# jhhung/kISS

Measured on AMD Instinct MI355X. Metric: bases/sec suffix_sort (chm13v2.0-size synthetic, k=256), higher is better.
Workload: dtype u8; 1 GPU; suffix_sort genome-like synthetic n=3117292070 k=256 (stand-in for chm13v2.0.fa, BASELINE.json configs[1]); PARALLEL_SORTING; text resident in HBM, SA left in HBM; n=3117292070, k=256, seed=2, parallelism=single GPU, lms=905939973, lms_rounds=9, tied_after_round0_item_rounds=184319413, big_segment_item_rounds=72866550, workspace_bytes=80357006484, induce_passes=47

## Files before the change

kiss_amd/csrc/induce.hip:

```cpp
#include "kiss_internal.hpp"
#include <cstdio>
#include <cstdlib>

namespace {

constexpr int IN_THREADS = 256;
#ifndef KISS_IN_ITEMS
#define KISS_IN_ITEMS 8
#endif
constexpr int IN_ITEMS = KISS_IN_ITEMS;
constexpr int IN_WAVES = IN_THREADS / 64;
constexpr int IN_TILE = IN_THREADS * IN_ITEMS;
constexpr int SM_THREADS = 1024;
constexpr uint64_t SMALL_MAX = 8192;

__device__ __forceinline__ uint32_t child_ctx(uint32_t parent)
{
    return (KISS_CTX_WORD(parent) >> 2) | (parent & KISS_CTX_TAINT);
}

__device__ __forceinline__ uint32_t cls_byte(uint32_t c)
{
    return (c & 3u) | ((c & 0x7FFFFFFEu) == 0u ? 4u : 0u);
}
static_assert(KISS_EMPTY_CTX == 1u && KISS_CTX_TAINT == 0x80000000u, "no bases <=> all bits but 0 and 31 clear");

struct LmsRemap {
    const uint32_t *fin;
    const uint32_t *npos;
    uint32_t E;
};

__device__ __forceinline__ uint32_t remap_below(const LmsRemap &rm, uint64_t j)
{
    uint32_t lo = 0, hi = rm.E;
    while (lo < hi) {
        const uint32_t mid = (lo + hi) >> 1;
        if ((uint64_t)rm.fin[mid] < j) lo = mid + 1;
        else hi = mid;
    }
    return lo;
}

__device__ __forceinline__ uint32_t remap_below_wave(const LmsRemap &rm, uint64_t j)
{
    if (rm.E > 256u) return remap_below(rm, j);
    uint32_t cnt = 0;
    for (uint32_t base = 0; base < rm.E; base += 64u) {
        const uint32_t i = base + lane_id();
        const bool lt = i < rm.E && (uint64_t)rm.fin[i] < j;
        const uint32_t c = (uint32_t)__popcll(__ballot(lt));
        cnt += c;
        if (c < 64u) break;
    }
    return cnt;
}

template <bool REMAP>
__device__ __forceinline__ uint32_t item_class(const uint64_t *__restrict__ pk, const uint32_t *srcP, uint32_t *srcC,
                                               int64_t idx, uint32_t emitmask, uint32_t *v_out, uint32_t *ctx_out,
                                               const LmsRemap &rm, uint8_t *srcK = nullptr)
{
    int64_t phys = idx;
    if (REMAP) {
        const uint32_t t = remap_below(rm, (uint64_t)idx);
        if (t < rm.E && (int64_t)rm.fin[t] == idx) {
            const uint32_t v = rm.npos[t];
            const uint32_t c = kiss_load_ctx(pk, v) | KISS_CTX_TAINT;
            *v_out = v;
            *ctx_out = c;
            const uint32_t pc = c & 3u;
            return (v != 0 && ((emitmask >> pc) & 1u)) ? pc : 4u;
        }
        phys = idx - (int64_t)t;
    }
    uint32_t c = srcC[phys];
    uint32_t v = srcP[phys];
    *v_out = v;
    if (KISS_CTX_WORD(c) <= KISS_EMPTY_CTX) {
        if (v == 0) {
            *ctx_out = c;
            return 4u;
        }
        c = kiss_load_ctx(pk, v) | (c & KISS_CTX_TAINT);
        srcC[phys] = c;
        if (srcK) srcK[phys] = (uint8_t)cls_byte(c);
    }
    *ctx_out = c;
    uint32_t pc = c & 3u;
    return ((emitmask >> pc) & 1u) ? pc : 4u;
}

template <bool REMAP>
__device__ __forceinline__ uint32_t item_class_only(const uint64_t *__restrict__ pk, const uint32_t *srcP, uint32_t *srcC,
                                                    int64_t idx, uint32_t emitmask, const LmsRemap &rm, uint8_t *srcK = nullptr)
{
    if (REMAP) {
        uint32_t v, c;
        return item_class<true>(pk, srcP, srcC, idx, emitmask, &v, &c, rm);
    }
    uint32_t c = srcC[idx];
    if (KISS_CTX_WORD(c) <= KISS_EMPTY_CTX) {
        const uint32_t v = srcP[idx];
        if (v == 0) return 4u;
        c = kiss_load_ctx(pk, v) | (c & KISS_CTX_TAINT);
        srcC[idx] = c;
        if (srcK) srcK[idx] = (uint8_t)cls_byte(c);
    }
    const uint32_t pc = c & 3u;
    return ((emitmask >> pc) & 1u) ? pc : 4u;
}

__device__ __forceinline__ uint32_t wave_scan_add(uint32_t x)
{
    x += (uint32_t)__builtin_amdgcn_update_dpp(0, (int)x, 0x111, 0xf, 0xf, true);
    x += (uint32_t)__builtin_amdgcn_update_dpp(0, (int)x, 0x112, 0xf, 0xf, true);
    x += (uint32_t)__builtin_amdgcn_update_dpp(0, (int)x, 0x114, 0xf, 0xf, true);
    x += (uint32_t)__builtin_amdgcn_update_dpp(0, (int)x, 0x118, 0xf, 0xf, true);
    x += (uint32_t)__builtin_amdgcn_update_dpp(0, (int)x, 0x142, 0xa, 0xf, true);
    x += (uint32_t)__builtin_amdgcn_update_dpp(0, (int)x, 0x143, 0xc, 0xf, true);
    return x;
}

template <bool REMAP>
__global__ __launch_bounds__(IN_THREADS) void k_induce_count(const uint64_t *__restrict__ pk, const uint32_t *srcP,
                                                            uint32_t *srcC, int64_t beg, uint64_t N, int dir,
                                                            uint32_t emitmask, uint32_t *__restrict__ counts,
                                                            uint64_t tiles, LmsRemap rm, uint8_t *srcK)
{
    if (blockIdx.x == 0 && threadIdx.x == 4) counts[4 * tiles] = 0;
    const uint64_t tile = (uint64_t)blockIdx.x * IN_WAVES + (threadIdx.x >> 6);
    if (tile >= tiles) return;
    struct __attribute__((packed, aligned(4))) U4 {
        uint32_t v[4];
    };
    constexpr int STEPS = IN_TILE / 256;
    const uint32_t lane = lane_id();
    const uint64_t t0 = tile * IN_TILE;
    uint64_t acc = 0;
    int64_t shift = 0;
    bool block = t0 + IN_TILE <= N;
    if (REMAP && block) {
        const uint32_t b0 = remap_below_wave(rm, (uint64_t)beg + t0);
        block = b0 == remap_below_wave(rm, (uint64_t)beg + t0 + IN_TILE);
        shift = (int64_t)b0;
    }
    bool counted = false;
    if (!REMAP && srcK != nullptr && block) {
        const int64_t lo_index = dir > 0 ? beg + (int64_t)t0 : beg - (int64_t)(t0 + IN_TILE - 1);
        const uint8_t *const A = srcK + lo_index;
        const uint32_t mis = (uint32_t)(reinterpret_cast<uintptr_t>(A) & 15u);
        const uint4 *const ap = reinterpret_cast<const uint4 *>(A - mis);
        static_assert(IN_TILE == 2048, "64 lanes x 2 x 16 bytes");
        uint32_t w[12];
        {
            const uint4 q0 = ap[lane], q1 = ap[64 + lane];
            w[0] = q0.x, w[1] = q0.y, w[2] = q0.z, w[3] = q0.w;
            w[4] = q1.x, w[5] = q1.y, w[6] = q1.z, w[7] = q1.w;
            w[8] = w[9] = w[10] = w[11] = 0x08080808u;
        }
        if (mis != 0 && lane == 0) {
            const uint4 q2 = ap[128];
            const uint32_t tail[4] = {q2.x, q2.y, q2.z, q2.w};
#pragma unroll
            for (int i = 0; i < 4; i++) {
                const int nb = (int)mis - 4 * i;
                const uint32_t lowmask = nb >= 4 ? 0xFFFFFFFFu : (nb <= 0 ? 0u : ~(0xFFFFFFFFu << (8 * nb)));
                w[i] = (w[i] & ~lowmask) | (0x08080808u & lowmask);
                w[8 + i] = (tail[i] & lowmask) | (0x08080808u & ~lowmask);
            }
        }
        uint32_t any = 0;
#pragma unroll
        for (int i = 0; i < 12; i++) any |= w[i];
        if (__ballot((any & 0x04040404u) != 0u) == 0ull) {
            uint32_t cnt8 = 0;
#pragma unroll
            for (int i = 0; i < 12; i++) {
#pragma unroll
                for (int e = 0; e < 4; e++) {
                    const uint32_t b = (w[i] >> (8 * e)) & 0xFFu;
                    const uint32_t pc = b & 3u;
                    cnt8 += ((emitmask >> pc) & ~(b >> 3) & 1u) << (pc << 3);
                }
            }
            acc = (uint64_t)((cnt8 & 0xFFu) | ((cnt8 & 0xFF00u) << 8)) | ((uint64_t)(((cnt8 >> 16) & 0xFFu) | ((cnt8 >> 8) & 0xFF0000u)) << 32);
            counted = true;
        }
    }
    if (counted) {
    } else if (block) {
        U4 t[STEPS];
        int64_t p0[STEPS];
        uint32_t least = 0xFFFFFFFFu;
#pragma unroll
        for (int q = 0; q < STEPS; q++) {
            const uint64_t i0 = t0 + (uint64_t)q * 256 + 4 * lane;
            p0[q] = (dir > 0 ? beg + (int64_t)i0 : beg - (int64_t)(i0 + 3)) - shift;
            t[q] = *reinterpret_cast<const U4 *>(srcC + p0[q]);
        }
#pragma unroll
        for (int q = 0; q < STEPS; q++)
#pragma unroll
            for (int e = 0; e < 4; e++) least = min(least, t[q].v[e] & 0x7FFFFFFEu);
        uint32_t cnt8 = 0;
        if (__ballot(least == 0u) == 0ull) {
#pragma unroll
            for (int q = 0; q < STEPS; q++) {
#pragma unroll
                for (int e = 0; e < 4; e++) {
                    const uint32_t pc = t[q].v[e] & 3u;
                    cnt8 += ((emitmask >> pc) & 1u) << (pc << 3);
                }
            }
        } else {
#pragma unroll
            for (int q = 0; q < STEPS; q++) {
#pragma unroll
                for (int e = 0; e < 4; e++) {
                    const uint32_t c = t[q].v[e];
                    uint32_t cls;
                    if (KISS_CTX_WORD(c) <= KISS_EMPTY_CTX) cls = item_class_only<false>(pk, srcP, srcC, p0[q] + e, emitmask, rm, REMAP ? nullptr : srcK);
                    else {
                        const uint32_t pc = c & 3u;
                        cls = ((emitmask >> pc) & 1u) ? pc : 4u;
                    }
                    cnt8 += (cls < 4u ? 1u : 0u) << ((cls & 3u) << 3);
                }
            }
        }
        static_assert(IN_TILE / 64 <= 255, "8-bit counters per lane");
        acc = (uint64_t)((cnt8 & 0xFFu) | ((cnt8 & 0xFF00u) << 8)) | ((uint64_t)(((cnt8 >> 16) & 0xFFu) | ((cnt8 >> 8) & 0xFF0000u)) << 32);
    } else {
        for (uint64_t i = t0 + lane; i < N && i < t0 + IN_TILE; i += 64) {
            const uint32_t cls = item_class_only<REMAP>(pk, srcP, srcC, beg + (int64_t)dir * (int64_t)i, emitmask, rm, REMAP ? nullptr : srcK);
            acc += cls < 4u ? 1ull << (16 * cls) : 0ull;
        }
    }
    const uint32_t slo = (uint32_t)__builtin_amdgcn_readlane((int)wave_scan_add((uint32_t)acc), 63);
    const uint32_t shi = (uint32_t)__builtin_amdgcn_readlane((int)wave_scan_add((uint32_t)(acc >> 32)), 63);
    acc = ((uint64_t)shi << 32) | slo;
    if (lane < 4) counts[(uint64_t)lane * tiles + tile] = (uint32_t)(acc >> (16 * lane)) & 0xFFFFu;
}

struct DstPos {
    int64_t p[4];
};

template <bool REMAP, int DIR>
__global__ __launch_bounds__(IN_THREADS) void k_induce_scatter(const uint64_t *__restrict__ pk, const uint32_t *srcP,
                                                              uint32_t *srcC, int64_t beg, uint64_t N,
                                                              uint32_t emitmask, const uint32_t *__restrict__ ex,
                                                              uint64_t tiles, DstPos dst, uint32_t *SA, uint32_t *CTX,
                                                              uint32_t *__restrict__ totals, LmsRemap rm,
                                                              uint8_t *CLS,
                                                              uint8_t *srcK)
{
    static_assert(IN_ITEMS == 8 && IN_WAVES == 4, "8-bit counters per thread, 4-bit ranks of a thread's items in one word");
    static_assert(!REMAP || DIR > 0, "the LMS list is read left to right only");
    __shared__ uint32_t wtot[IN_WAVES][2];
    __shared__ __attribute__((aligned(16))) uint32_t stP[IN_TILE];
    __shared__ __attribute__((aligned(16))) uint32_t stC[IN_TILE];
    if (blockIdx.x == 0 && threadIdx.x < 4) totals[threadIdx.x] = ex[(uint64_t)(threadIdx.x + 1) * tiles] - ex[(uint64_t)threadIdx.x * tiles];
    const int wave = threadIdx.x >> 6;
    struct __attribute__((packed, aligned(4))) U4 {
        uint32_t v[4];
    };
    const uint64_t i0 = (uint64_t)blockIdx.x * IN_TILE + (uint64_t)threadIdx.x * IN_ITEMS;
    uint32_t vv[IN_ITEMS], cc[IN_ITEMS];
    uint32_t okm = 0;
    uint32_t loc = 0;
    uint32_t cnt8 = 0;
    auto take = [&](int e, uint32_t pc, uint32_t ok) {
        const uint32_t sh = pc << 3;
        loc |= ((cnt8 >> sh) & 15u) << (4 * e);
        cnt8 += ok << sh;
        okm |= ok << e;
    };
    int64_t shift = 0;
    bool block = i0 + IN_ITEMS <= N;
    if (REMAP) {
        const uint64_t tj = (uint64_t)beg + (uint64_t)blockIdx.x * IN_TILE;
        const uint32_t t0 = remap_below_wave(rm, tj), t1 = remap_below_wave(rm, tj + IN_TILE);
        if (t0 == t1) shift = (int64_t)t0;
        else if (block) {
            const uint32_t b0 = remap_below(rm, (uint64_t)beg + i0);
            block = b0 == remap_below(rm, (uint64_t)beg + i0 + IN_ITEMS);
            shift = (int64_t)b0;
        }
    }
    if (block) {
        const int64_t p0 = (DIR > 0 ? beg + (int64_t)i0 : beg - (int64_t)(i0 + IN_ITEMS - 1)) - shift;
        uint32_t bp[IN_ITEMS], bc[IN_ITEMS];
#pragma unroll
        for (int q = 0; q < IN_ITEMS / 4; q++) {
            const U4 tp = *reinterpret_cast<const U4 *>(srcP + p0 + 4 * q);
            const U4 tcw = *reinterpret_cast<const U4 *>(srcC + p0 + 4 * q);
#pragma unroll
            for (int e = 0; e < 4; e++) {
                bp[4 * q + e] = tp.v[e];
                bc[4 * q + e] = tcw.v[e];
            }
        }
        uint32_t least = 0xFFFFFFFFu;
#pragma unroll
        for (int e = 0; e < IN_ITEMS; e++) least = min(least, bc[e] & 0x7FFFFFFEu);
        static_assert(KISS_EMPTY_CTX == 1u && KISS_CTX_TAINT == 0x80000000u, "no bases <=> all bits but 0 and 31 clear");
        constexpr int last = IN_ITEMS - 1;
        if (__ballot(least == 0u) == 0ull) {
#pragma unroll
            for (int e = 0; e < IN_ITEMS; e++) {
                const int a = DIR > 0 ? e : last - e;
                const uint32_t pc = bc[a] & 3u;
                take(e, pc, (emitmask >> pc) & 1u);
                vv[e] = bp[a];
                cc[e] = bc[a];
            }
        } else {
#pragma unroll
            for (int e = 0; e < IN_ITEMS; e++) {
                const int a = DIR > 0 ? e : last - e;
                uint32_t v = bp[a], c = bc[a];
                if (KISS_CTX_WORD(c) <= KISS_EMPTY_CTX) {
                    const uint32_t cls = item_class<false>(pk, srcP, srcC, p0 + a, emitmask, &v, &c, rm, REMAP ? nullptr : srcK);
                    take(e, cls & 3u, cls < 4u ? 1u : 0u);
                } else {
                    const uint32_t pc = c & 3u;
                    take(e, pc, (emitmask >> pc) & 1u);
                }
                vv[e] = v;
                cc[e] = c;
            }
        }
    } else {
#pragma unroll
        for (int e = 0; e < IN_ITEMS; e++) {
            const uint64_t i = i0 + (uint64_t)e;
            uint32_t cls = 4u, v = 0, c = 0;
            if (i < N) cls = item_class<REMAP>(pk, srcP, srcC, beg + (int64_t)DIR * (int64_t)i, emitmask, &v, &c, rm, REMAP ? nullptr : srcK);
            take(e, cls & 3u, cls < 4u ? 1u : 0u);
            vv[e] = v;
            cc[e] = c;
        }
    }
    const uint32_t mylo = (cnt8 & 0xFFu) | ((cnt8 & 0xFF00u) << 8), myhi = ((cnt8 >> 16) & 0xFFu) | ((cnt8 >> 8) & 0xFF0000u);
    const uint32_t inlo = wave_scan_add(mylo), inhi = wave_scan_add(myhi);
    if (lane_id() == 63) {
        wtot[wave][0] = inlo;
        wtot[wave][1] = inhi;
    }
    __syncthreads();
    uint32_t tlo = 0, thi = 0, olo = 0, ohi = 0;
#pragma unroll
    for (int w = 0; w < IN_WAVES; w++) {
        const uint32_t a = wtot[w][0], b = wtot[w][1];
        tlo += a;
        thi += b;
        if (w < wave) {
            olo += a;
            ohi += b;
        }
    }
    const uint32_t c1 = tlo & 0xFFFFu, c2 = c1 + (tlo >> 16), c3 = c2 + (thi & 0xFFFFu), total = c3 + (thi >> 16);
    const uint32_t blo = (c1 << 16) + olo + (inlo - mylo), bhi = (c2 | (c3 << 16)) + ohi + (inhi - myhi);
#pragma unroll
    for (int e = 0; e < IN_ITEMS; e++) {
        if ((okm >> e) & 1u) {
            const uint32_t pc = cc[e] & 3u;
            const uint32_t base = __builtin_amdgcn_perm(bhi, blo, 0x0c0c0100u + pc * 0x0202u);
            const uint32_t li = base + ((loc >> (4 * e)) & 15u);
            stP[li] = vv[e] - 1u;
            stC[li] = child_ctx(cc[e]);
        }
    }
    __syncthreads();
    int64_t db[4];
    {
        const uint32_t cs[4] = {0u, c1, c2, c3};
#pragma unroll
        for (int k = 0; k < 4; k++) {
            const uint32_t toff = ex[(uint64_t)k * tiles + blockIdx.x] - ex[(uint64_t)k * tiles];
            db[k] = dst.p[k] + (int64_t)DIR * ((int64_t)toff - (int64_t)cs[k]);
        }
    }
    for (uint32_t l0 = threadIdx.x * 4u; l0 < total; l0 += IN_THREADS * 4u) {
        const uint32_t cls = (l0 >= c1 ? 1u : 0u) + (l0 >= c2 ? 1u : 0u) + (l0 >= c3 ? 1u : 0u);
        const uint32_t cend = cls == 0 ? c1 : (cls == 1 ? c2 : (cls == 2 ? c3 : total));
        if (l0 + 4u <= cend) {
            const int64_t dbk = cls == 0 ? db[0] : (cls == 1 ? db[1] : (cls == 2 ? db[2] : db[3]));
            const int64_t d0 = dbk + (int64_t)DIR * (int64_t)l0;
            const uint4 sp = *reinterpret_cast<const uint4 *>(stP + l0), sc = *reinterpret_cast<const uint4 *>(stC + l0);
            U4 wp, wc;
            if (DIR > 0) {
                wp.v[0] = sp.x, wp.v[1] = sp.y, wp.v[2] = sp.z, wp.v[3] = sp.w;
                wc.v[0] = sc.x, wc.v[1] = sc.y, wc.v[2] = sc.z, wc.v[3] = sc.w;
            } else {
                wp.v[0] = sp.w, wp.v[1] = sp.z, wp.v[2] = sp.y, wp.v[3] = sp.x;
                wc.v[0] = sc.w, wc.v[1] = sc.z, wc.v[2] = sc.y, wc.v[3] = sc.x;
            }
            const int64_t lo = DIR > 0 ? d0 : d0 - 3;
            *reinterpret_cast<U4 *>(SA + lo) = wp;
            *reinterpret_cast<U4 *>(CTX + lo) = wc;
            if (CLS) {
                struct __attribute__((packed, aligned(1))) B4 {
                    uint32_t v;
                };
                reinterpret_cast<B4 *>(CLS + lo)->v =
                    cls_byte(wc.v[0]) | (cls_byte(wc.v[1]) << 8) | (cls_byte(wc.v[2]) << 16) | (cls_byte(wc.v[3]) << 24);
            }
        } else {
            for (uint32_t li = l0; li < l0 + 4u && li < total; li++) {
                const uint32_t c2_ = (li >= c1 ? 1u : 0u) + (li >= c2 ? 1u : 0u) + (li >= c3 ? 1u : 0u);
                const int64_t dbk = c2_ == 0 ? db[0] : (c2_ == 1 ? db[1] : (c2_ == 2 ? db[2] : db[3]));
                const int64_t d = dbk + (int64_t)DIR * (int64_t)li;
                SA[d] = stP[li];
                CTX[d] = stC[li];
                if (CLS) CLS[d] = (uint8_t)cls_byte(stC[li]);
            }
        }
    }
}

constexpr uint32_t IN_SPIN_LIMIT = 1u << 22;
static_assert(IN_WAVES == 4, "wave c of a partition tile walks class c");

__device__ __forceinline__ uint32_t in_lookback(uint64_t *__restrict__ d, uint32_t tile, uint32_t mine, uint64_t tag,
                                                uint32_t *__restrict__ err)
{
    const uint32_t lane = lane_id();
    constexpr uint64_t TAGMASK = 0x3FFFFFFFull << 32;
    if (tile == 0) {
        if (lane == 0) __hip_atomic_store(&d[0], (2ull << 62) | tag | mine, __ATOMIC_RELAXED, __HIP_MEMORY_SCOPE_AGENT);
        return 0u;
    }
    if (lane == 0) __hip_atomic_store(&d[tile], (1ull << 62) | tag | mine, __ATOMIC_RELAXED, __HIP_MEMORY_SCOPE_AGENT);
    uint32_t excl = 0, spins = 0;
    int64_t base = (int64_t)tile;
    for (;;) {
        const int64_t t = base - 1 - (int64_t)lane;
        uint64_t v = t >= 0 ? __hip_atomic_load(&d[t], __ATOMIC_RELAXED, __HIP_MEMORY_SCOPE_AGENT) : ((2ull << 62) | tag);
        if ((v & TAGMASK) != tag) v = 0;
        const uint32_t st = (uint32_t)(v >> 62);
        const uint64_t incl = __ballot(st == 2u), ready = __ballot(st != 0u);
        const uint32_t first = incl ? (uint32_t)__builtin_ctzll(incl) : 64u;
        const uint64_t need = first >= 63u ? ~0ull : ((2ull << first) - 1ull);
        if ((ready & need) != need) {
            if (++spins > IN_SPIN_LIMIT) {
                if (lane == 0) *err = 1;
                break;
            }
            __builtin_amdgcn_s_sleep(1);
            continue;
        }
        uint32_t a = lane <= first ? (uint32_t)v : 0u;
#pragma unroll
        for (int dd = 32; dd >= 1; dd >>= 1) a += __shfl_xor(a, dd, 64);
        excl += a;
        if (first < 64u) break;
        base -= 64;
    }
    if (lane == 0) __hip_atomic_store(&d[tile], (2ull << 62) | tag | (uint64_t)(uint32_t)(excl + mine), __ATOMIC_RELAXED, __HIP_MEMORY_SCOPE_AGENT);
    return excl;
}

template <bool REMAP>
__global__ __launch_bounds__(IN_THREADS) void k_induce_onepass(const uint64_t *__restrict__ pk, const uint32_t *srcP,
                                                              uint32_t *srcC, int64_t beg, uint64_t N, int dir,
                                                              uint32_t emitmask, uint64_t tiles, DstPos dst, uint32_t *SA,
                                                              uint32_t *CTX, uint32_t *__restrict__ totals, LmsRemap rm,
                                                              uint64_t *__restrict__ desc, uint64_t desc_stride,
                                                              uint32_t *__restrict__ ctl, uint32_t ticket_base, uint64_t epoch)
{
    __shared__ uint32_t wtot[IN_WAVES][4];
    __shared__ uint32_t s_tile;
    __shared__ uint32_t s_excl[4];
    __shared__ uint32_t stP[IN_TILE], stC[IN_TILE];
    if (threadIdx.x == 0) s_tile = atomicAdd(&ctl[2], 1u) - ticket_base;
    __syncthreads();
    const uint32_t tile = s_tile;
    if (tile >= tiles) return;
    const int wave = threadIdx.x >> 6;
    struct __attribute__((packed, aligned(4))) U4 {
        uint32_t v[4];
    };
    const uint64_t i0 = (uint64_t)tile * IN_TILE + (uint64_t)threadIdx.x * IN_ITEMS;
    uint32_t vv[IN_ITEMS], cc[IN_ITEMS], rr[IN_ITEMS];
    uint32_t cnt[4] = {0, 0, 0, 0};
    int64_t shift = 0;
    bool block = i0 + IN_ITEMS <= N;
    if (REMAP) {
        const uint64_t tj = (uint64_t)beg + (uint64_t)tile * IN_TILE;
        const uint32_t t0 = remap_below_wave(rm, tj), t1 = remap_below_wave(rm, tj + IN_TILE);
        if (t0 == t1) shift = (int64_t)t0;
        else if (block) {
            const uint32_t b0 = remap_below(rm, (uint64_t)beg + i0);
            block = b0 == remap_below(rm, (uint64_t)beg + i0 + IN_ITEMS);
            shift = (int64_t)b0;
        }
    }
    if (block) {
        const int64_t p0 = (dir > 0 ? beg + (int64_t)i0 : beg - (int64_t)(i0 + IN_ITEMS - 1)) - shift;
        uint32_t bp[IN_ITEMS], bc[IN_ITEMS];
#pragma unroll
        for (int q = 0; q < IN_ITEMS / 4; q++) {
            const U4 tp = *reinterpret_cast<const U4 *>(srcP + p0 + 4 * q);
            const U4 tcw = *reinterpret_cast<const U4 *>(srcC + p0 + 4 * q);
#pragma unroll
            for (int e = 0; e < 4; e++) {
                bp[4 * q + e] = tp.v[e];
                bc[4 * q + e] = tcw.v[e];
            }
        }
#pragma unroll
        for (int e = 0; e < IN_ITEMS; e++) {
            const int a = dir > 0 ? e : IN_ITEMS - 1 - e;
            uint32_t v = bp[a], c = bc[a], cls;
            if (KISS_CTX_WORD(c) <= KISS_EMPTY_CTX) cls = item_class<false>(pk, srcP, srcC, p0 + a, emitmask, &v, &c, rm);
            else {
                const uint32_t pc = c & 3u;
                cls = ((emitmask >> pc) & 1u) ? pc : 4u;
            }
            uint32_t local = 0;
#pragma unroll
            for (int k = 0; k < 4; k++) {
                if (cls == (uint32_t)k) local = cnt[k];
                cnt[k] += cls == (uint32_t)k ? 1u : 0u;
            }
            vv[e] = v;
            cc[e] = c;
            rr[e] = (cls << 28) | local;
        }
    } else {
#pragma unroll
        for (int e = 0; e < IN_ITEMS; e++) {
            const uint64_t i = i0 + (uint64_t)e;
            uint32_t cls = 4u, v = 0, c = 0;
            if (i < N) cls = item_class<REMAP>(pk, srcP, srcC, beg + (int64_t)dir * (int64_t)i, emitmask, &v, &c, rm);
            uint32_t local = 0;
#pragma unroll
            for (int k = 0; k < 4; k++) {
                if (cls == (uint32_t)k) local = cnt[k];
                cnt[k] += cls == (uint32_t)k ? 1u : 0u;
            }
            vv[e] = v;
            cc[e] = c;
// ... 654 lines not shown
```

Baseline: 46.59 billion bases/s.

## Restructure induce count kernel with SWAR class counting and lazy pending refresh

Splits the induce count kernel into byte-tile, word-tile and partial-tile paths. The byte path now counts classes with SWAR bit arithmetic (four byte-lane accumulators summed by multiplication) instead of per-byte extract-and-shift loops, and loads the misaligned tail across four lanes rather than lane 0 alone. Tiles that contain stale entries no longer fall back to per-item reclassification of the whole tile. Only the pending items, kept in a bitmask, are refreshed in a ballot loop, and the counts are corrected incrementally. This saves ALU work and avoids full-tile fallback, at the cost of extra control flow and register use.

```diff
diff --git a/kiss_amd/csrc/induce.hip b/kiss_amd/csrc/induce.hip
--- a/kiss_amd/csrc/induce.hip
+++ b/kiss_amd/csrc/induce.hip
@@ -1,4 +1,5 @@
 #include "kiss_internal.hpp"
+#include "induce_count.hpp"
 #include <cstdio>
 #include <cstdlib>
 
@@ -122,6 +123,145 @@
     return x;
 }
 
+
+template <int SH>
+__device__ __forceinline__ uint32_t refresh_pending(const uint64_t *__restrict__ pk, const uint32_t *srcP, uint32_t *srcC,
+                                                    uint8_t *srcK, uint64_t pend, int64_t base, int64_t step, int64_t tail,
+                                                    uint32_t cnt8, bool counted_before)
+{
+    while (__ballot(pend != 0ull) != 0ull) {
+        if (pend != 0ull) {
+            const uint32_t b = (uint32_t)__ffsll((unsigned long long)pend) - 1u;
+            pend &= pend - 1ull;
+            const int64_t idx = b < 32u ? base + step * (int64_t)(b >> SH) + (int64_t)(b & ((1u << SH) - 1u)) : tail + (int64_t)(b - 32u);
+            const uint32_t old = srcC[idx];
+            if (counted_before) cnt8 -= 1u << ((old & 3u) << 3);
+            const uint32_t v = srcP[idx];
+            if (v != 0u) {
+                const uint32_t c = kiss_load_ctx(pk, v) | (old & KISS_CTX_TAINT);
+                srcC[idx] = c;
+                if (srcK) srcK[idx] = (uint8_t)cls_byte(c);
+                cnt8 += 1u << ((c & 3u) << 3);
+            }
+        }
+    }
+    return cnt8;
+}
+
+__device__ __forceinline__ void put_counts(uint32_t *__restrict__ counts, uint64_t tiles, uint64_t tile, uint32_t cnt8)
+{
+    const uint32_t lane = lane_id();
+    const uint32_t lo = (cnt8 & 0xFFu) | ((cnt8 & 0xFF00u) << 8), hi = ((cnt8 >> 16) & 0xFFu) | ((cnt8 >> 8) & 0xFF0000u);
+    const uint32_t slo = (uint32_t)__builtin_amdgcn_readlane((int)wave_scan_add(lo), 63);
+    const uint32_t shi = (uint32_t)__builtin_amdgcn_readlane((int)wave_scan_add(hi), 63);
+    if (lane < 4) counts[(uint64_t)lane * tiles + tile] = (((lane & 2u) ? shi : slo) >> (16u * (lane & 1u))) & 0xFFFFu;
+}
+
+__device__ __forceinline__ void count_byte_tile(const uint64_t *__restrict__ pk, const uint32_t *srcP, uint32_t *srcC,
+                                                uint8_t *srcK, int64_t beg, int dir, uint32_t emitmask,
+                                                uint32_t *__restrict__ counts, uint64_t tiles, uint64_t tile)
+{
+    static_assert(IN_TILE == 2048, "64 lanes x 2 x 16 bytes");
+    const uint32_t lane = lane_id();
+    const uint64_t t0 = tile * IN_TILE;
+    const int64_t lo_index = dir > 0 ? beg + (int64_t)t0 : beg - (int64_t)(t0 + IN_TILE - 1);
+    const uint32_t mis = (uint32_t)__builtin_amdgcn_readfirstlane((int)(reinterpret_cast<uintptr_t>(srcK + lo_index) & 15u));
+    const int64_t first = lo_index - (int64_t)mis;
+    const uint4 *const ap = reinterpret_cast<const uint4 *>(srcK + first);
+    uint32_t w[9];
+    {
+        const uint4 q0 = ap[lane], q1 = ap[64 + lane];
+        w[0] = q0.x, w[1] = q0.y, w[2] = q0.z, w[3] = q0.w;
+        w[4] = q1.x, w[5] = q1.y, w[6] = q1.z, w[7] = q1.w;
+        w[8] = 0x08080808u;
+    }
+    if (mis != 0u) {
+        if (lane < 4u) w[8] = reinterpret_cast<const uint32_t *>(ap + 128)[lane];
+#pragma unroll
+        for (int i = 0; i < 4; i++) {
+            const int nb = (int)mis - 4 * i;
+            const uint32_t lowmask = nb >= 4 ? 0xFFFFFFFFu : (nb <= 0 ? 0u : ~(0xFFFFFFFFu << (8 * (nb & 3))));
+            if (lane == 0u) w[i] = (w[i] & ~lowmask) | (0x08080808u & lowmask);
+        }
+        const int nb = (int)mis - 4 * (int)lane;
+        const uint32_t lowmask = nb >= 4 ? 0xFFFFFFFFu : (nb <= 0 ? 0u : ~(0xFFFFFFFFu << (8 * (nb & 3))));
+        w[8] = (w[8] & lowmask) | (0x08080808u & ~lowmask);
+    }
+    KissClsAcc acc = {{0u, 0u, 0u, 0u}};
+    uint32_t any = 0;
+#pragma unroll
+    for (int i = 0; i < 8; i++) {
+        kiss_cls_acc_add(acc, w[i]);
+        any |= w[i];
+    }
+    if (mis != 0u) {
+        kiss_cls_acc_add(acc, w[8]);
+        any |= w[8];
+    }
+    uint32_t cnt8 = kiss_cls_acc_sum(acc);
+    if (__ballot((any & 0x04040404u) != 0u) != 0ull) {
+        uint64_t pend = 0;
+#pragma unroll
+        for (int i = 0; i < 9; i++) {
+            const uint32_t p = (w[i] >> 2) & ~(w[i] >> 3) & 0x01010101u;
+            pend |= (uint64_t)(((p * 0x00204081u) >> 21) & 0xFu) << (4 * i);
+        }
+        cnt8 = refresh_pending<4>(pk, srcP, srcC, srcK, pend, first + 16 * (int64_t)lane, 1024, first + 2048 + 4 * (int64_t)lane,
+                                  cnt8, false);
+    }
+    put_counts(counts, tiles, tile, kiss_cls_emit(cnt8, emitmask));
+}
+
+__device__ __forceinline__ void count_word_tile(const uint64_t *__restrict__ pk, const uint32_t *srcP, uint32_t *srcC, int64_t beg,
+                                                int dir, uint32_t emitmask, uint32_t *__restrict__ counts, uint64_t tiles,
+                                                uint64_t tile, int64_t shift)
+{
+    struct __attribute__((packed, aligned(4))) U4 {
+        uint32_t v[4];
+    };
+    constexpr int STEPS = IN_TILE / 256;
+    static_assert(STEPS * 4 == 32, "one bit per item of a lane in the low half of refresh_pending's mask");
+    static_assert(IN_TILE / 64 <= 255, "8-bit counters per lane");
+    const uint64_t i0 = tile * IN_TILE + 4 * lane_id();
+    const int64_t p0 = (dir > 0 ? beg + (int64_t)i0 : beg - (int64_t)(i0 + 3)) - shift;
+    const int64_t pstep = dir > 0 ? 256 : -256;
+    U4 t[STEPS];
+#pragma unroll
+    for (int q = 0; q < STEPS; q++) t[q] = *reinterpret_cast<const U4 *>(srcC + (p0 + q * pstep));
+    uint32_t cnt8 = 0, least = 0xFFFFFFFFu;
+#pragma unroll
+    for (int q = 0; q < STEPS; q++) {
+#pragma unroll
+        for (int e = 0; e < 4; e++) {
+            cnt8 += 1u << ((t[q].v[e] << 3) & 31u);
+            least = min(least, t[q].v[e] & 0x7FFFFFFEu);
+        }
+    }
+    if (__ballot(least == 0u) != 0ull) {
+        uint32_t pend = 0;
+#pragma unroll
+        for (int q = 0; q < STEPS; q++)
+#pragma unroll
+            for (int e = 0; e < 4; e++) pend |= ((t[q].v[e] & 0x7FFFFFFEu) == 0u ? 1u : 0u) << (4 * q + e);
+        cnt8 = refresh_pending<2>(pk, srcP, srcC, nullptr, (uint64_t)pend, p0, pstep, 0, cnt8, true);
+    }
+    put_counts(counts, tiles, tile, kiss_cls_emit(cnt8, emitmask));
+}
+
+template <bool REMAP>
+__device__ __forceinline__ void count_partial_tile(const uint64_t *__restrict__ pk, const uint32_t *srcP, uint32_t *srcC, int64_t beg,
+                                                   uint64_t N, int dir, uint32_t emitmask, uint32_t *__restrict__ counts,
+                                                   uint64_t tiles, uint64_t tile, const LmsRemap &rm, uint8_t *srcK)
+{
+    const uint64_t t0 = tile * IN_TILE;
+    uint32_t cnt8 = 0;
+    for (uint64_t i = t0 + lane_id(); i < N && i < t0 + IN_TILE; i += 64) {
+        const uint32_t cls = item_class_only<REMAP>(pk, srcP, srcC, beg + (int64_t)dir * (int64_t)i, emitmask, rm, REMAP ? nullptr : srcK);
+        cnt8 += (cls < 4u ? 1u : 0u) << ((cls & 3u) << 3);
+    }
+    put_counts(counts, tiles, tile, cnt8);
+}
+
 template <bool REMAP>
 __global__ __launch_bounds__(IN_THREADS) void k_induce_count(const uint64_t *__restrict__ pk, const uint32_t *srcP,
                                                             uint32_t *srcC, int64_t beg, uint64_t N, int dir,
@@ -129,15 +269,10 @@
                                                             uint64_t tiles, LmsRemap rm, uint8_t *srcK)
 {
     if (blockIdx.x == 0 && threadIdx.x == 4) counts[4 * tiles] = 0;
-    const uint64_t tile = (uint64_t)blockIdx.x * IN_WAVES + (threadIdx.x >> 6);
+    const uint32_t wave = (uint32_t)__builtin_amdgcn_readfirstlane((int)(threadIdx.x >> 6));
+    const uint64_t tile = (uint64_t)blockIdx.x * IN_WAVES + wave;
     if (tile >= tiles) return;
-    struct __attribute__((packed, aligned(4))) U4 {
-        uint32_t v[4];
-    };
-    constexpr int STEPS = IN_TILE / 256;
-    const uint32_t lane = lane_id();
     const uint64_t t0 = tile * IN_TILE;
-    uint64_t acc = 0;
     int64_t shift = 0;
     bool block = t0 + IN_TILE <= N;
     if (REMAP && block) {
@@ -145,102 +280,9 @@
         block = b0 == remap_below_wave(rm, (uint64_t)beg + t0 + IN_TILE);
         shift = (int64_t)b0;
     }
-    bool counted = false;
-    if (!REMAP && srcK != nullptr && block) {
-        const int64_t lo_index = dir > 0 ? beg + (int64_t)t0 : beg - (int64_t)(t0 + IN_TILE - 1);
-        const uint8_t *const A = srcK + lo_index;
-        const uint32_t mis = (uint32_t)(reinterpret_cast<uintptr_t>(A) & 15u);
-        const uint4 *const ap = reinterpret_cast<const uint4 *>(A - mis);
-        static_assert(IN_TILE == 2048, "64 lanes x 2 x 16 bytes");
-        uint32_t w[12];
-        {
-            const uint4 q0 = ap[lane], q1 = ap[64 + lane];
-            w[0] = q0.x, w[1] = q0.y, w[2] = q0.z, w[3] = q0.w;
-            w[4] = q1.x, w[5] = q1.y, w[6] = q1.z, w[7] = q1.w;
-            w[8] = w[9] = w[10] = w[11] = 0x08080808u;
-        }
-        if (mis != 0 && lane == 0) {
-            const uint4 q2 = ap[128];
-            const uint32_t tail[4] = {q2.x, q2.y, q2.z, q2.w};
-#pragma unroll
-            for (int i = 0; i < 4; i++) {
-                const int nb = (int)mis - 4 * i;
-                const uint32_t lowmask = nb >= 4 ? 0xFFFFFFFFu : (nb <= 0 ? 0u : ~(0xFFFFFFFFu << (8 * nb)));
-                w[i] = (w[i] & ~lowmask) | (0x08080808u & lowmask);
-                w[8 + i] = (tail[i] & lowmask) | (0x08080808u & ~lowmask);
-            }
-        }
-        uint32_t any = 0;
-#pragma unroll
-        for (int i = 0; i < 12; i++) any |= w[i];
-        if (__ballot((any & 0x04040404u) != 0u) == 0ull) {
-            uint32_t cnt8 = 0;
-#pragma unroll
-            for (int i = 0; i < 12; i++) {
-#pragma unroll
-                for (int e = 0; e < 4; e++) {
-                    const uint32_t b = (w[i] >> (8 * e)) & 0xFFu;
-                    const uint32_t pc = b & 3u;
-                    cnt8 += ((emitmask >> pc) & ~(b >> 3) & 1u) << (pc << 3);
-                }
-            }
-            acc = (uint64_t)((cnt8 & 0xFFu) | ((cnt8 & 0xFF00u) << 8)) | ((uint64_t)(((cnt8 >> 16) & 0xFFu) | ((cnt8 >> 8) & 0xFF0000u)) << 32);
-            counted = true;
-        }
-    }
-    if (counted) {
-    } else if (block) {
-        U4 t[STEPS];
-        int64_t p0[STEPS];
-        uint32_t least = 0xFFFFFFFFu;
-#pragma unroll
-        for (int q = 0; q < STEPS; q++) {
-            const uint64_t i0 = t0 + (uint64_t)q * 256 + 4 * lane;
-            p0[q] = (dir > 0 ? beg + (int64_t)i0 : beg - (int64_t)(i0 + 3)) - shift;
-            t[q] = *reinterpret_cast<const U4 *>(srcC + p0[q]);
-        }
-#pragma unroll
-        for (int q = 0; q < STEPS; q++)
-#pragma unroll
-            for (int e = 0; e < 4; e++) least = min(least, t[q].v[e] & 0x7FFFFFFEu);
-        uint32_t cnt8 = 0;
-        if (__ballot(least == 0u) == 0ull) {
-#pragma unroll
-            for (int q = 0; q < STEPS; q++) {
-#pragma unroll
-                for (int e = 0; e < 4; e++) {
-                    const uint32_t pc = t[q].v[e] & 3u;
-                    cnt8 += ((emitmask >> pc) & 1u) << (pc << 3);
-                }
-            }
-        } else {
-#pragma unroll
-            for (int q = 0; q < STEPS; q++) {
-#pragma unroll
-                for (int e = 0; e < 4; e++) {
-                    const uint32_t c = t[q].v[e];
-                    uint32_t cls;
-                    if (KISS_CTX_WORD(c) <= KISS_EMPTY_CTX) cls = item_class_only<false>(pk, srcP, srcC, p0[q] + e, emitmask, rm, REMAP ? nullptr : srcK);
-                    else {
-                        const uint32_t pc = c & 3u;
-                        cls = ((emitmask >> pc) & 1u) ? pc : 4u;
-                    }
-                    cnt8 += (cls < 4u ? 1u : 0u) << ((cls & 3u) << 3);
-                }
-            }
-        }
-        static_assert(IN_TILE / 64 <= 255, "8-bit counters per lane");
-        acc = (uint64_t)((cnt8 & 0xFFu) | ((cnt8 & 0xFF00u) << 8)) | ((uint64_t)(((cnt8 >> 16) & 0xFFu) | ((cnt8 >> 8) & 0xFF0000u)) << 32);
-    } else {
-        for (uint64_t i = t0 + lane; i < N && i < t0 + IN_TILE; i += 64) {
-            const uint32_t cls = item_class_only<REMAP>(pk, srcP, srcC, beg + (int64_t)dir * (int64_t)i, emitmask, rm, REMAP ? nullptr : srcK);
-            acc += cls < 4u ? 1ull << (16 * cls) : 0ull;
-        }
-    }
-    const uint32_t slo = (uint32_t)__builtin_amdgcn_readlane((int)wave_scan_add((uint32_t)acc), 63);
-    const uint32_t shi = (uint32_t)__builtin_amdgcn_readlane((int)wave_scan_add((uint32_t)(acc >> 32)), 63);
-    acc = ((uint64_t)shi << 32) | slo;
-    if (lane < 4) counts[(uint64_t)lane * tiles + tile] = (uint32_t)(acc >> (16 * lane)) & 0xFFFFu;
+    if (!block) count_partial_tile<REMAP>(pk, srcP, srcC, beg, N, dir, emitmask, counts, tiles, tile, rm, srcK);
+    else if (!REMAP && srcK != nullptr) count_byte_tile(pk, srcP, srcC, srcK, beg, dir, emitmask, counts, tiles, tile);
+    else count_word_tile(pk, srcP, srcC, beg, dir, emitmask, counts, tiles, tile, shift);
 }
 
 struct DstPos {
diff --git a/kiss_amd/csrc/induce_count.hpp b/kiss_amd/csrc/induce_count.hpp
--- /dev/null
+++ b/kiss_amd/csrc/induce_count.hpp
@@ -0,0 +1,46 @@
+#pragma once
+#include <cstdint>
+
+#if defined(__HIPCC__)
+#define KISS_CNT_HD __host__ __device__ __forceinline__
+#else
+#define KISS_CNT_HD inline
+#endif
+
+constexpr int KISS_CNT_MAX_WORDS = 63;
+
+struct KissClsAcc {
+    uint32_t a[4];
+};
+
+KISS_CNT_HD void kiss_cls_acc_add(KissClsAcc &acc, uint32_t w)
+{
+    const uint32_t ones = 0x01010101u;
+    const uint32_t lo = w, hi = w >> 1;
+    const uint32_t live = ~(w >> 2) & ~(w >> 3) & ones;
+    acc.a[0] += live & ~lo & ~hi;
+    acc.a[1] += live & lo & ~hi;
+    acc.a[2] += live & ~lo & hi;
+    acc.a[3] += live & lo & hi;
+}
+
+KISS_CNT_HD uint32_t kiss_cls_acc_sum(const KissClsAcc &acc)
+{
+    const uint32_t ones = 0x01010101u;
+    return ((acc.a[0] * ones) >> 24) | (((acc.a[1] * ones) >> 24) << 8) | (((acc.a[2] * ones) >> 24) << 16) |
+           ((acc.a[3] * ones) & 0xFF000000u);
+}
+
+KISS_CNT_HD uint32_t kiss_cls_emit(uint32_t cnt8, uint32_t emitmask)
+{
+    const uint32_t keep = ((emitmask & 1u) ? 0x000000FFu : 0u) | ((emitmask & 2u) ? 0x0000FF00u : 0u) |
+                          ((emitmask & 4u) ? 0x00FF0000u : 0u) | ((emitmask & 8u) ? 0xFF000000u : 0u);
+    return cnt8 & keep;
+}
+
+KISS_CNT_HD uint32_t kiss_cls_count_packed(const uint32_t *w, int nwords, uint32_t emitmask)
+{
+    KissClsAcc acc = {{0u, 0u, 0u, 0u}};
+    for (int i = 0; i < nwords; i++) kiss_cls_acc_add(acc, w[i]);
+    return kiss_cls_emit(kiss_cls_acc_sum(acc), emitmask);
+}
```

Result: faster. 47.40 billion bases/s, median of 6 (+1.8%).
